# xuanjiangliu/robotic-discovery-platform

Hardware: AMD Instinct MI355X
Metric: U-Net train imgs/sec at 256×256 (1/2/4/8 GPU); e2e frames/sec + p50 latency (higher is better)
Workload: dtype bf16; 1 GPU; model=UNet(3,1) bilinear decoder, 17.26M params, global_batch=64, per_gpu_batch=64, image_size=256, parallelism=dp1, impl=native, optimizer=Adam(lr=1e-4), loss=bce, sync_bn=False, hipgraph=False

## Files before the change

### csrc/conv_wgrad.hip

```cpp
#include "common.h"
#include <algorithm>
#include <stdlib.h>
#include <string.h>

struct WgradArgs {
  const u16* x1;
  const u16* x2;
  uint32_t xbytes1, xbytes2;
  int C1, C2, pitch1, pitch2;
  const u16* dy;
  uint32_t dybytes;
  int dypitch;
  float* slab;
  int H, W, M, Cout, Cin;
  int taps, packed;
  int ncols, ncols_pad;
  int colTiles, coutTiles, splits;
  int pix_per_split;
  uint32_t fw_m, fw_s, fh_m, fh_s;
  int uH2 = 0, uW2 = 0, uoy = 0, uox = 0;
};

RDP_DEV int swz(int p) { return (((p >> 1) & 1) << 1) | (((p >> 3) & 1) << 2); }

// ... 582 lines not shown
  }
}


extern "C" int rdp_conv_wgrad(const void* x1, const void* x2, long xbytes1, long xbytes2, int C1, int C2, int pitch1,
                              int pitch2, const void* dy, long dybytes, int dypitch, float* slab, long slab_elems,
                              float* out, int accumulate, int N, int H, int W, int Cout, int taps, int packed,
                              int cin_real, int splits, int variant, hipStream_t s) {
  WgradArgs a;
  a.x1 = (const u16*)x1; a.x2 = (const u16*)x2;
  a.xbytes1 = (uint32_t)xbytes1; a.xbytes2 = (uint32_t)xbytes2;
  a.C1 = C1; a.C2 = C2; a.pitch1 = pitch1; a.pitch2 = pitch2;
  a.dy = (const u16*)dy; a.dybytes = (uint32_t)dybytes; a.dypitch = dypitch;
  a.slab = slab; a.H = H; a.W = W; a.M = N * H * W; a.Cout = Cout;
  a.taps = taps; a.packed = packed;
  if (packed) {
    if (C1 != 8 || C2 != 0 || taps != 9) return -1;
    a.Cin = 8; a.ncols = 72;
  } else {
    if (C1 % 64 || C2 % 64) return -1;
    a.Cin = C1 + C2; a.ncols = taps * a.Cin;
  }
  if (Cout % 64) return -1;
  if (xbytes1 >= (1l << 31) || xbytes2 >= (1l << 31) || dybytes >= (1l << 31)) return -1;
  const bool halo_ok = !packed && taps == 9 && (W % 64 == 0 || (W >= 32 && 64 % W == 0 && (H * W) % 64 == 0)) &&
                       variant != 4;
  if (variant == 5 && !(!packed && taps == 9 && (W % 64 == 0 || (W >= 8 && 64 % W == 0 && (H * W) % 64 == 0))))
    return -1;
  if (halo_ok || variant == 5) {
    WgradHaloArgs h;
    h.x1 = a.x1; h.x2 = a.x2; h.xbytes1 = a.xbytes1; h.xbytes2 = a.xbytes2;
    h.C1 = C1; h.C2 = C2; h.pitch1 = pitch1; h.pitch2 = pitch2;
    h.dy = a.dy; h.dybytes = a.dybytes; h.dypitch = dypitch;
    h.slab = slab; h.H = H; h.W = W; h.Cout = Cout; h.ncols = 9 * a.Cin;
    const int BN = Cout % 128 == 0 ? 128 : 64;
    h.cinTiles = a.Cin / 64; h.coutTiles = Cout / BN;
    const int tiles = h.cinTiles * h.coutTiles;
    h.nseg = a.M / 64;
    const int target = BN == 64 ? 512 : 256;
    int sp = std::max(1, (target + tiles - 1) / tiles);
    sp = std::min(sp, std::max(1, h.nseg));
    const long per_split = (long)Cout * h.ncols;
    sp = (int)std::min<long>(sp, slab_elems / per_split);
    if (sp < 1) return -2;
    h.segs_per_split = (h.nseg + sp - 1) / sp;
    h.splits = (h.nseg + h.segs_per_split - 1) / h.segs_per_split;
    if ((long)h.splits * per_split * 4l >= (1l << 31)) return -3;
    h.slab_bytes = (uint32_t)(h.splits * per_split * 4l);
    FastDiv fw = make_fastdiv(W), fh = make_fastdiv(H);
    h.fw_m = fw.m; h.fw_s = fw.s; h.fh_m = fh.m; h.fh_s = fh.s;
    const int nblk = tiles * h.splits;
    if (variant == 0 && W % 64 == 0 && BN == 64) {
      WgradRingArgs g;
      g.x1 = h.x1; g.x2 = h.x2; g.xbytes1 = h.xbytes1; g.xbytes2 = h.xbytes2;
      g.C1 = C1; g.C2 = C2; g.pitch1 = pitch1; g.pitch2 = pitch2;
      g.dy = h.dy; g.dybytes = h.dybytes; g.dypitch = dypitch;
      g.slab = slab; g.slab_bytes = h.slab_bytes; g.H = H; g.W = W; g.Cout = Cout; g.ncols = h.ncols;
      g.cinTiles = h.cinTiles; g.coutTiles = h.coutTiles; g.splits = h.splits;
      g.pos_per_split = h.segs_per_split; g.npos = h.nseg; g.WS = W / 64;
      FastDiv fs = make_fastdiv(W / 64);
      g.fh_m = fh.m; g.fh_s = fh.s; g.fs_m = fs.m; g.fs_s = fs.s;
      hipLaunchKernelGGL((conv_wgrad_ring_kernel<64>), dim3(nblk), dim3(256), 0, s, g);
    } else {
      const bool mr = W < 64;
      if (BN == 128 && mr) hipLaunchKernelGGL((conv_wgrad_halo_kernel<128, true>), dim3(nblk), dim3(512), 0, s, h);
      else if (BN == 128) hipLaunchKernelGGL((conv_wgrad_halo_kernel<128, false>), dim3(nblk), dim3(512), 0, s, h);
      else if (mr) hipLaunchKernelGGL((conv_wgrad_halo_kernel<64, true>), dim3(nblk), dim3(256), 0, s, h);
      else hipLaunchKernelGGL((conv_wgrad_halo_kernel<64, false>), dim3(nblk), dim3(256), 0, s, h);
    }
    rdp_wgrad_reduce(slab, out, h.splits, Cout, h.ncols, 9, a.Cin, a.Cin, accumulate, s);
    return h.splits;
  }
  a.colTiles = (a.ncols + 255) / 256;
  a.ncols_pad = a.colTiles * 256;
  a.coutTiles = Cout / 64;
  if (splits < 1) splits = 1;
  int pps = (a.M + splits - 1) / splits;
  pps = (pps + 63) / 64 * 64;
  a.pix_per_split = pps;
  a.splits = (a.M + pps - 1) / pps;
  if ((long)a.splits * Cout * a.ncols_pad > slab_elems) return -2;
  if ((long)a.splits * Cout * a.ncols_pad * 4l >= (1l << 31)) return -3;
  FastDiv fw = make_fastdiv(W), fh = make_fastdiv(H);
  a.fw_m = fw.m; a.fw_s = fw.s; a.fh_m = fh.m; a.fh_s = fh.s;
  const int nblk = a.colTiles * a.coutTiles * a.splits;
  if (packed) hipLaunchKernelGGL((conv_wgrad_kernel<true>), dim3(nblk), dim3(512), 0, s, a);
  else hipLaunchKernelGGL((conv_wgrad_kernel<false>), dim3(nblk), dim3(512), 0, s, a);
  rdp_wgrad_reduce(slab, out, a.splits, Cout, a.ncols_pad, taps, packed ? 8 : a.Cin, packed ? cin_real : a.Cin,
                   accumulate, s);
  return a.splits;
}

extern "C" int rdp_conv_wgrad_upT(const void* du, long dubytes, int C, int dupitch, int H2, int W2, int oy, int ox,
                                  const void* x, long xbytes, int Cin, int xpitch, int N, int h, int w, float* slab,
                                  long slab_elems, float* out, int accumulate, int splits, hipStream_t s) {
  if (C % 64 || Cin % 64 || oy < 0 || ox < 0 || 2 * h + oy > H2 || 2 * w + ox > W2) return -1;
  if (dubytes >= (1l << 31) || xbytes >= (1l << 31)) return -1;
  WgradArgs a;
  a.x1 = (const u16*)du; a.x2 = nullptr; a.xbytes1 = (uint32_t)dubytes; a.xbytes2 = 0;
  a.C1 = C; a.C2 = 0; a.pitch1 = dupitch; a.pitch2 = dupitch;
  a.dy = (const u16*)x; a.dybytes = (uint32_t)xbytes; a.dypitch = xpitch;
  a.slab = slab; a.H = h; a.W = w; a.M = N * h * w; a.Cout = Cin;
  a.taps = 4; a.packed = 0; a.Cin = C; a.ncols = 4 * C;
  a.uH2 = H2; a.uW2 = W2; a.uoy = oy; a.uox = ox;
  a.colTiles = (a.ncols + 255) / 256;
  a.ncols_pad = a.colTiles * 256;
  a.coutTiles = Cin / 64;
  if (splits < 1) splits = 1;
  int pps = (a.M + splits - 1) / splits;
  pps = (pps + 63) / 64 * 64;
  a.pix_per_split = pps;
  a.splits = (a.M + pps - 1) / pps;
  if ((long)a.splits * a.Cout * a.ncols_pad > slab_elems) return -2;
  if ((long)a.splits * a.Cout * a.ncols_pad * 4l >= (1l << 31)) return -3;
  FastDiv fw = make_fastdiv(w), fh = make_fastdiv(h);
  a.fw_m = fw.m; a.fw_s = fw.s; a.fh_m = fh.m; a.fh_s = fh.s;
  const int nblk = a.colTiles * a.coutTiles * a.splits;
  hipLaunchKernelGGL((conv_wgrad_kernel<false, true>), dim3(nblk), dim3(512), 0, s, a);
  rdp_wgrad_reduce(slab, out, a.splits, Cin, a.ncols_pad, 4, C, C, accumulate, s);
  return a.splits;
}

struct FirstWgradArgs {
  const u16* x;
  uint32_t xbytes;
  int xpitch;
  const u16* da;
  uint32_t dabytes;
  int dapitch;
  const u16* y;
  uint32_t ybytes;
  int ypitch;
  const float* coef;
  const float* coef2;
  float* slab;
  uint32_t slab_bytes;
  int H, W, M, pix_per_split;
  uint32_t fw_m, fw_s, fh_m, fh_s;
};
constexpr int FWG_NCOLS = 80;

RDP_DEV void fw_unpack8(const uint4& v, float* f) {
  const uint32_t w[4] = {v.x, v.y, v.z, v.w};
#pragma unroll
  for (int i = 0; i < 4; ++i) {
    f[2 * i] = __uint_as_float(w[i] << 16);
    f[2 * i + 1] = __uint_as_float(w[i] & 0xffff0000u);
  }
}

__global__ __launch_bounds__(256, 2) void wgrad_first_bn_kernel(const FirstWgradArgs a) {
  constexpr int SUB = 64 * 128;
  constexpr int BUF = 3 * SUB;
  __shared__ __attribute__((aligned(16))) char smem[2 * BUF];
  const int lane = threadIdx.x & 63;
  const int wave = __builtin_amdgcn_readfirstlane(threadIdx.x >> 6);
  const int split = (int)xcd_remap(blockIdx.x, gridDim.x);
  const int pbeg = split * a.pix_per_split;
  const int nks = max(0, min(a.M, pbeg + a.pix_per_split) - pbeg) / 64;
  const auto rx = make_rsrc(a.x, a.xbytes);
  const auto rda = make_rsrc(a.da, a.dabytes);
  const auto ry = make_rsrc(a.y, a.ybytes);

  const int tc = threadIdx.x & 7, tr0 = threadIdx.x >> 3;
  float ss[8], hh[8], cA[8], cB[8], cK[8];
#pragma unroll
  for (int k = 0; k < 8; ++k) {
    const int c = 8 * tc + k;
    ss[k] = a.coef[128 + c]; hh[k] = a.coef[192 + c];
    cA[k] = a.coef2[c]; cB[k] = a.coef2[64 + c]; cK[k] = a.coef2[128 + c];
  }
  uint4 vd[2], vy[2];
  auto load_dz = [&](int ks) {
#pragma unroll
    for (int u = 0; u < 2; ++u) {
      const int m = pbeg + ks * 64 + tr0 + 32 * u;
      vd[u] = bload16(rda, (uint32_t)(m * a.dapitch + 8 * tc) * 2u);
      vy[u] = bload16(ry, (uint32_t)(m * a.ypitch + 8 * tc) * 2u);
    }
  };
  auto store_dz = [&](char* buf) {
#pragma unroll
    for (int u = 0; u < 2; ++u) {
      const int p = tr0 + 32 * u;
      float fd[8], fy[8];
      fw_unpack8(vd[u], fd);
      fw_unpack8(vy[u], fy);
      uint32_t o[4];
#pragma unroll
      for (int k = 0; k < 8; k += 2) {
        const float g0 = fmaf(fy[k], ss[k], hh[k]) > 0.f ? fd[k] : 0.f;
        const float g1 = fmaf(fy[k + 1], ss[k + 1], hh[k + 1]) > 0.f ? fd[k + 1] : 0.f;
        o[k / 2] = pack2bf(fmaf(cA[k], g0, fmaf(cB[k], fy[k], cK[k])),
                           fmaf(cA[k + 1], g1, fmaf(cB[k + 1], fy[k + 1], cK[k + 1])));
      }
      *(uint4*)(buf + 2 * SUB + p * 128 + 16 * (tc ^ swz(p))) = make_uint4(o[0], o[1], o[2], o[3]);
    }
  };
  const int rowl = lane >> 3, cpos = lane & 7;
  auto issue_x = [&](int ks, char* buf) {
#pragma unroll
    for (int t = 0; t < 4; ++t) {
      const int s = wave * 4 + t, sub = s >> 3, pj = s & 7;
      const int p = pj * 8 + rowl;
      const int g = cpos ^ swz(p);
      const int m = pbeg + ks * 64 + p;
      const uint32_t q = fdiv2((uint32_t)m, a.fw_m, a.fw_s);
      const int w = m - (int)q * a.W;
      const int h = (int)q - (int)fdiv2(q, a.fh_m, a.fh_s) * a.H;
      const int tap = sub * 8 + g;
      const int dr = tap / 3 - 1, ds = tap % 3 - 1;
      const bool ok = (tap < 9) & inb(h + dr, a.H) & inb(w + ds, a.W);
      const uint32_t off = ok ? (uint32_t)((m + dr * a.W + ds) * a.xpitch) * 2u : RDP_OOB;
      dma16_async(rx, (lds_void*)(buf + sub * SUB + pj * 1024), off);
    }
  };

  f32x4 acc[5];
#pragma unroll
  for (int i = 0; i < 5; ++i) acc[i] = f32x4{0.f, 0.f, 0.f, 0.f};
  const int tg = lane >> 4, tq = (lane >> 2) & 3, tpp = lane & 3;
  typedef __attribute__((address_space(3))) bf16x4 lds_v4;

  if (nks > 0) {
    load_dz(0);
    issue_x(0, smem);
    store_dz(smem);
  }
  for (int ks = 0; ks < nks; ++ks) {
    asm volatile("s_waitcnt vmcnt(0) lgkmcnt(0)" ::: "memory");
    raw_barrier();
    const char* cur = smem + (ks & 1) * BUF;
    char* nxt = smem + ((ks + 1) & 1) * BUF;
    const bool more = ks + 1 < nks;
    if (more) {
      load_dz(ks + 1);
      issue_x(ks + 1, nxt);
    }
#pragma unroll
    for (int hf = 0; hf < 2; ++hf) {
      const int p0 = 32 * hf + 8 * tg + tq;
      const int sw0 = swz(p0), sw1 = swz(p0 + 4);
      const int ro0 = p0 * 128 + 8 * (tpp & 1), ro1 = ro0 + 4 * 128;
      auto frag = [&](const char* base, int i) {
        const int c = 2 * i + (tpp >> 1);
        const bf16x4 b0 = __builtin_amdgcn_ds_read_tr16_b64_v4i16((lds_v4*)(base + ro0 + 16 * (c ^ sw0)));
        const bf16x4 b1 = __builtin_amdgcn_ds_read_tr16_b64_v4i16((lds_v4*)(base + ro1 + 16 * (c ^ sw1)));
        return __builtin_shufflevector(b0, b1, 0, 1, 2, 3, 4, 5, 6, 7);
      };
      const bf16x8 fb = frag(cur + 2 * SUB, wave);
      bf16x8 fa[5];
#pragma unroll
      for (int i = 0; i < 4; ++i) fa[i] = frag(cur, i);
      fa[4] = frag(cur + SUB, 0);
#pragma unroll
      for (int i = 0; i < 5; ++i) acc[i] = __builtin_amdgcn_mfma_f32_16x16x32_bf16(fa[i], fb, acc[i], 0, 0, 0);
    }
    if (more) store_dz(nxt);
  }

  const auto rs = make_rsrc(a.slab, a.slab_bytes);
  const int co = 16 * wave + (lane & 15);
#pragma unroll
  for (int i = 0; i < 5; ++i) {
    const int col = 16 * i + 4 * (lane >> 4);
    const uint32_t off = (uint32_t)(((long)split * 64 + co) * FWG_NCOLS + col) * 4u;
    uint4 v;
    v.x = __float_as_uint(acc[i][0]); v.y = __float_as_uint(acc[i][1]);
    v.z = __float_as_uint(acc[i][2]); v.w = __float_as_uint(acc[i][3]);
    bstore16(rs, off, v);
  }
}

extern "C" int rdp_wgrad_first_bn(const void* x, long xbytes, int xpitch, const void* da, long dabytes, int dapitch,
                                  const void* y, long ybytes, int ypitch, const float* coef, const float* coef2,
                                  float* slab, long slab_elems, float* out, int accumulate, int N, int H, int W,
                                  int cin_real, int splits, hipStream_t s) {
  const long M = (long)N * H * W;
  if (M % 64 || cin_real > 8 || cin_real < 1) return -1;
  if (xbytes >= (1l << 31) || dabytes >= (1l << 31) || ybytes >= (1l << 31)) return -1;
  if (xpitch % 8 || dapitch % 8 || ypitch % 8) return -1;
  splits = (int)std::max(1L, std::min<long>(splits, M / 64));
  long pps = (M + splits - 1) / splits;
  pps = (pps + 63) / 64 * 64;
  splits = (int)((M + pps - 1) / pps);
  const long per_split = 64l * FWG_NCOLS;
  if ((long)splits * per_split > slab_elems) return -2;
  if ((long)splits * per_split * 4l >= (1l << 31)) return -3;
  FirstWgradArgs a;
  a.x = (const u16*)x; a.xbytes = (uint32_t)xbytes; a.xpitch = xpitch;
  a.da = (const u16*)da; a.dabytes = (uint32_t)dabytes; a.dapitch = dapitch;
  a.y = (const u16*)y; a.ybytes = (uint32_t)ybytes; a.ypitch = ypitch;
  a.coef = coef; a.coef2 = coef2;
  a.slab = slab; a.slab_bytes = (uint32_t)(splits * per_split * 4l);
  a.H = H; a.W = W; a.M = (int)M; a.pix_per_split = (int)pps;
  FastDiv fw = make_fastdiv(W), fh = make_fastdiv(H);
  a.fw_m = fw.m; a.fw_s = fw.s; a.fh_m = fh.m; a.fh_s = fh.s;
  hipLaunchKernelGGL(wgrad_first_bn_kernel, dim3(splits), dim3(256), 0, s, a);
  rdp_wgrad_reduce(slab, out, splits, 64, FWG_NCOLS, 9, 8, cin_real, accumulate, s);
  return splits;
}

extern "C" long rdp_conv_wgrad_slab_elems(int N, int H, int W, int Cin, int Cout, int taps, int packed, int splits) {
  const int ncols = packed ? 72 : taps * Cin;
  const int ncols_pad = (ncols + 255) / 256 * 256;
  const long M = (long)N * H * W;
  long pps = (M + splits - 1) / splits;
  pps = (pps + 63) / 64 * 64;
  const long sp = (M + pps - 1) / pps;
  return sp * Cout * ncols_pad;
}

extern "C" long rdp_conv_wgrad_halo_slab_elems(int N, int H, int W, int Cin, int Cout) {
  const long M = (long)N * H * W;
  const bool halo = Cin % 64 == 0 && Cout % 64 == 0 && (W % 64 == 0 || (W >= 32 && 64 % W == 0 && (H * W) % 64 == 0));
  if (!halo) return 0;
  const int BN = Cout % 128 == 0 ? 128 : 64;
  const long tiles = (long)(Cin / 64) * (Cout / BN);
  const long target = BN == 64 ? 512 : 256;
  long hsp = std::max<long>(1, (target + tiles - 1) / tiles);
  hsp = std::min<long>(hsp, std::max<long>(1, M / 64));
  return hsp * Cout * 9L * Cin;
}
```

### csrc/pool_up.hip

```cpp
#include "common.h"
#include <algorithm>

RDP_DEV void unpack8f(const uint4& v, float* f) {
  const uint32_t w[4] = {v.x, v.y, v.z, v.w};
#pragma unroll
  for (int k = 0; k < 4; ++k) {
    f[2 * k] = __uint_as_float(w[k] << 16);
    f[2 * k + 1] = __uint_as_float(w[k] & 0xffff0000u);
  }
}
RDP_DEV uint4 pack8f(const float* f) {
  uint4 v;
  v.x = pack2bf(f[0], f[1]);
  v.y = pack2bf(f[2], f[3]);
  v.z = pack2bf(f[4], f[5]);
  v.w = pack2bf(f[6], f[7]);
  return v;
}

__global__ void maxpool2_fwd_kernel(const u16* __restrict__ x, int xpitch, u16* __restrict__ out, int opitch, int N,
                                    int H, int W, int C) {
  const int Ho = H / 2, Wo = W / 2, CG = C >> 3;
  const long total = (long)N * Ho * Wo * CG;
  for (long it = blockIdx.x * (long)blockDim.x + threadIdx.x; it < total; it += (long)gridDim.x * blockDim.x) {
    const int g = it % CG;
    const long po = it / CG;
    const int wo = po % Wo;
    const long t = po / Wo;
    const int ho = t % Ho, n = t / Ho;
    const long p00 = ((long)n * H + 2 * ho) * W + 2 * wo;
    const int c = g * 8;
    float v[4][8];
    unpack8f(*(const uint4*)(x + p00 * xpitch + c), v[0]);
    unpack8f(*(const uint4*)(x + (p00 + 1) * xpitch + c), v[1]);
    unpack8f(*(const uint4*)(x + (p00 + W) * xpitch + c), v[2]);
    unpack8f(*(const uint4*)(x + (p00 + W + 1) * xpitch + c), v[3]);
    float o[8];
#pragma unroll
    for (int k = 0; k < 8; ++k) {
      float m = v[0][k];
#pragma unroll
      for (int q = 1; q < 4; ++q)
        if (v[q][k] > m || isnan(v[q][k])) m = v[q][k];
      o[k] = m;
    }
    *(uint4*)(out + po * opitch + c) = pack8f(o);
  }
}

__global__ void maxpool2_bwd_kernel(const u16* __restrict__ dp, int dppitch, const u16* __restrict__ x, int xpitch,
                                    const u16* __restrict__ dskip, int dspitch, u16* __restrict__ dx, int dxpitch,
                                    int N, int H, int W, int C) {
  const int Ho = H / 2, Wo = W / 2, CG = C >> 3;
  const int Hc = (H + 1) / 2, Wc = (W + 1) / 2;
  const long total = (long)N * Hc * Wc * CG;
  for (long it = blockIdx.x * (long)blockDim.x + threadIdx.x; it < total; it += (long)gridDim.x * blockDim.x) {
    const int g = it % CG;
    const long pw = it / CG;
    const int wc = pw % Wc;
    const long t = pw / Wc;
    const int hc = t % Hc, n = t / Hc;
    const int c = g * 8;
    const bool pooled = hc < Ho && wc < Wo;
    float v[4][8], d[8], o[4][8];
    int idx[8];
    if (pooled) {
      const long p00 = ((long)n * H + 2 * hc) * W + 2 * wc;
      unpack8f(*(const uint4*)(x + p00 * xpitch + c), v[0]);
      unpack8f(*(const uint4*)(x + (p00 + 1) * xpitch + c), v[1]);
      unpack8f(*(const uint4*)(x + (p00 + W) * xpitch + c), v[2]);
      unpack8f(*(const uint4*)(x + (p00 + W + 1) * xpitch + c), v[3]);
      const long po = ((long)n * Ho + hc) * Wo + wc;
      unpack8f(*(const uint4*)(dp + po * dppitch + c), d);
#pragma unroll
      for (int k = 0; k < 8; ++k) {
        float m = v[0][k];
        int id = 0;
#pragma unroll
        for (int q = 1; q < 4; ++q)
          if (v[q][k] > m || isnan(v[q][k])) { m = v[q][k]; id = q; }
        idx[k] = id;
      }
    }
#pragma unroll
    for (int q = 0; q < 4; ++q) {
      const int hh = 2 * hc + (q >> 1), ww = 2 * wc + (q & 1);
      if (hh >= H || ww >= W) continue;
      const long p = ((long)n * H + hh) * W + ww;
      float s[8];
      if (dskip) unpack8f(*(const uint4*)(dskip + p * dspitch + c), s);
      else {
#pragma unroll
        for (int k = 0; k < 8; ++k) s[k] = 0.f;
      }
#pragma unroll
      for (int k = 0; k < 8; ++k) o[q][k] = s[k] + ((pooled && idx[k] == q) ? d[k] : 0.f);
      *(uint4*)(dx + p * dxpitch + c) = pack8f(o[q]);
    }
  }
}

RDP_DEV void ld8f(const float* p, float* f) {
  const float4 a = *(const float4*)p, b = *(const float4*)(p + 4);
  f[0] = a.x; f[1] = a.y; f[2] = a.z; f[3] = a.w; f[4] = b.x; f[5] = b.y; f[6] = b.z; f[7] = b.w;
}

__global__ __launch_bounds__(256) void bn_relu_apply_pool_kernel(const u16* __restrict__ y, int ypitch,
                                                                 u16* __restrict__ a, int apitch,
                                                                 u16* __restrict__ pool, int ppitch,
                                                                 const float* __restrict__ coef, int N, int H, int W,
                                                                 int C) {
  const int CG = C >> 3, RPB = 256 / CG;
  const int g = threadIdx.x & (CG - 1), r = threadIdx.x / CG;
  const int c = g * 8;
  float ss[8], hh[8];
  ld8f(coef + 2 * C + c, ss);
  ld8f(coef + 3 * C + c, hh);
  const int Ho = H / 2, Wo = W / 2, Hc = (H + 1) / 2, Wc = (W + 1) / 2;
  const int nwin = N * Hc * Wc;
  for (int wi = blockIdx.x * RPB + r; wi < nwin; wi += gridDim.x * RPB) {
    const int wc = wi % Wc, t = wi / Wc;
    const int hc = t % Hc, n = t / Hc;
    uint4 v[4];
    bool ok[4];
    long px[4];
#pragma unroll
    for (int q = 0; q < 4; ++q) {
      const int h = 2 * hc + (q >> 1), w = 2 * wc + (q & 1);
      ok[q] = h < H && w < W;
      px[q] = ((long)n * H + h) * W + w;
      if (ok[q]) v[q] = *(const uint4*)(y + px[q] * ypitch + c);
    }
    float av[4][8];
#pragma unroll
    for (int q = 0; q < 4; ++q) {
      if (!ok[q]) continue;
      float f[8];
      unpack8f(v[q], f);
#pragma unroll
      for (int k = 0; k < 8; ++k) f[k] = fmaxf(fmaf(f[k], ss[k], hh[k]), 0.f);
      const uint4 o = pack8f(f);
      if (a) *(uint4*)(a + px[q] * apitch + c) = o;
      unpack8f(o, av[q]);
    }
    if (hc < Ho && wc < Wo) {
      float o[8];
#pragma unroll
      for (int k = 0; k < 8; ++k) {
        float m = av[0][k];
#pragma unroll
        for (int q = 1; q < 4; ++q)
          if (av[q][k] > m || isnan(av[q][k])) m = av[q][k];
        o[k] = m;
      }
      *(uint4*)(pool + (((long)n * Ho + hc) * Wo + wc) * ppitch + c) = pack8f(o);
    }
  }
}

__global__ __launch_bounds__(256) void maxpool2_bwd_bn_reduce_kernel(
    const u16* __restrict__ dp, int dppitch, const u16* __restrict__ dskip,
    int dspitch, u16* __restrict__ dx, int dxpitch, const u16* __restrict__ y, int ypitch,
    const float* __restrict__ coef, int N, int H, int W, int C, float* __restrict__ partial) {
  extern __shared__ __attribute__((aligned(16))) float sred[];
  const int CG = C >> 3, RPB = 256 / CG;
  const int g = threadIdx.x & (CG - 1), r = threadIdx.x / CG;
  const int c = g * 8;
  float mean[8], inv[8], ss[8], hh[8];
  ld8f(coef + c, mean);
  ld8f(coef + C + c, inv);
  ld8f(coef + 2 * C + c, ss);
  ld8f(coef + 3 * C + c, hh);
  float sg[8], sgx[8];
#pragma unroll
  for (int k = 0; k < 8; ++k) { sg[k] = 0.f; sgx[k] = 0.f; }
  const int Ho = H / 2, Wo = W / 2, Hc = (H + 1) / 2, Wc = (W + 1) / 2;
  const int nwin = N * Hc * Wc;
  for (int wi = blockIdx.x * RPB + r; wi < nwin; wi += gridDim.x * RPB) {
    const int wc = wi % Wc, t = wi / Wc;
    const int hc = t % Hc, n = t / Hc;
    const bool pooled = hc < Ho && wc < Wo;
    bool ok[4];
    long px[4];
    uint4 vs[4], vy[4], vd;
#pragma unroll
    for (int q = 0; q < 4; ++q) {
      const int h = 2 * hc + (q >> 1), w = 2 * wc + (q & 1);
      ok[q] = h < H && w < W;
      px[q] = ((long)n * H + h) * W + w;
      if (ok[q]) {
        vy[q] = *(const uint4*)(y + px[q] * ypitch + c);
        vs[q] = dskip ? *(const uint4*)(dskip + px[q] * dspitch + c) : make_uint4(0, 0, 0, 0);
      }
    }
    if (pooled) vd = *(const uint4*)(dp + (((long)n * Ho + hc) * Wo + wc) * dppitch + c);
    int idx[8];
    float d[8];
    if (pooled) {
      float v[4][8];
#pragma unroll
      for (int q = 0; q < 4; ++q) {
        float f[8];
        unpack8f(vy[q], f);
#pragma unroll
        for (int k = 0; k < 8; ++k) f[k] = fmaxf(fmaf(f[k], ss[k], hh[k]), 0.f);
        unpack8f(pack8f(f), v[q]);
      }
      unpack8f(vd, d);
#pragma unroll
      for (int k = 0; k < 8; ++k) {
        float m = v[0][k];
        int id = 0;
#pragma unroll
        for (int q = 1; q < 4; ++q)
          if (v[q][k] > m || isnan(v[q][k])) { m = v[q][k]; id = q; }
        idx[k] = id;
      }
    }
#pragma unroll
    for (int q = 0; q < 4; ++q) {
      if (!ok[q]) continue;
      float sk[8], o[8], fy[8];
      unpack8f(vs[q], sk);
#pragma unroll
      for (int k = 0; k < 8; ++k) o[k] = sk[k] + ((pooled && idx[k] == q) ? d[k] : 0.f);
      const uint4 ov = pack8f(o);
      *(uint4*)(dx + px[q] * dxpitch + c) = ov;
      unpack8f(ov, o);
      unpack8f(vy[q], fy);
#pragma unroll
      for (int k = 0; k < 8; ++k) {
        const float gg = fmaf(fy[k], ss[k], hh[k]) > 0.f ? o[k] : 0.f;
        sg[k] += gg;
        sgx[k] += gg * (fy[k] - mean[k]) * inv[k];
      }
    }
  }
#pragma unroll
  for (int k = 0; k < 8; ++k) {
    sred[(r * C + c + k) * 2] = sg[k];
    sred[(r * C + c + k) * 2 + 1] = sgx[k];
  }
  __syncthreads();
  for (int cc = threadIdx.x; cc < C; cc += 256) {
    float a0 = 0.f, a1 = 0.f;
    for (int q = 0; q < RPB; ++q) { a0 += sred[(q * C + cc) * 2]; a1 += sred[(q * C + cc) * 2 + 1]; }
    partial[(size_t)blockIdx.x * 2 * C + cc] = a0;
    partial[(size_t)blockIdx.x * 2 * C + C + cc] = a1;
  }
}

struct UpGeom {
  int N, hin, win, Hout, Wout, oy, ox, C;
  float rh, rw;
};

RDP_DEV void up_src(int u, int in, float r, int& i0, int& i1, float& l1) {
  const float s = r * (float)u;
  i0 = (int)s;
  i1 = i0 + (i0 < in - 1 ? 1 : 0);
  l1 = s - (float)i0;
}

RDP_DEV void bn_relu8(float* v, const float* sc, const float* sh) {
#pragma unroll
  for (int k = 0; k < 8; ++k) v[k] = bf2f(f2bf(fmaxf(fmaf(v[k], sc[k], sh[k]), 0.f)));
}

__global__ __launch_bounds__(256) void upsample2_fwd_taps_kernel(const u16* __restrict__ x, int xpitch,
                                                                 u16* __restrict__ out, int opitch, UpGeom g, int lcg,
                                                                 int nchunk, const float* __restrict__ coef) {
  const int CG = 1 << lcg;
  const int items = g.N * g.Hout * nchunk;
  for (int it = blockIdx.x; it < items; it += gridDim.x) {
    const int row = it / nchunk, q = it - row * nchunk;
    const int n = row / g.Hout, Y = row - n * g.Hout;
    const int t = q * 256 + threadIdx.x;
    const int X = t >> lcg, c = (t & (CG - 1)) * 8;
    if (X >= g.Wout) continue;
    const int uy = Y - g.oy, ux = X - g.ox;
    float o[8];
    if (uy < 0 || ux < 0 || uy >= 2 * g.hin || ux >= 2 * g.win) {
#pragma unroll
      for (int k = 0; k < 8; ++k) o[k] = 0.f;
    } else {
      int y0, y1, x0, x1;
      float ly, lx;
      up_src(uy, g.hin, g.rh, y0, y1, ly);
      up_src(ux, g.win, g.rw, x0, x1, lx);
      const long base = (long)n * g.hin;
      float a[8], b[8], cc[8], d[8];
      unpack8f(*(const uint4*)(x + ((base + y0) * g.win + x0) * xpitch + c), a);
      unpack8f(*(const uint4*)(x + ((base + y0) * g.win + x1) * xpitch + c), b);
      unpack8f(*(const uint4*)(x + ((base + y1) * g.win + x0) * xpitch + c), cc);
      unpack8f(*(const uint4*)(x + ((base + y1) * g.win + x1) * xpitch + c), d);
      if (coef) {
        float sc[8], sh[8];
#pragma unroll
        for (int k = 0; k < 8; ++k) { sc[k] = coef[2 * g.C + c + k]; sh[k] = coef[3 * g.C + c + k]; }
        bn_relu8(a, sc, sh); bn_relu8(b, sc, sh); bn_relu8(cc, sc, sh); bn_relu8(d, sc, sh);
      }
      const float hy = 1.f - ly, hx = 1.f - lx;
#pragma unroll
      for (int k = 0; k < 8; ++k) o[k] = hy * (hx * a[k] + lx * b[k]) + ly * (hx * cc[k] + lx * d[k]);
    }
    *(uint4*)(out + ((long)row * g.Wout + X) * opitch + c) = pack8f(o);
  }
}

RDP_DEV void up_hrow(const u16* __restrict__ x, long rowbase, int x0, int x1, int xpitch, int c, float hx,
                     float lx, const float* __restrict__ coef, int C, float* h) {
  float a[8], b[8];
  unpack8f(*(const uint4*)(x + (rowbase + x0) * xpitch + c), a);
  unpack8f(*(const uint4*)(x + (rowbase + x1) * xpitch + c), b);
  if (coef) {
    float sc[8], sh[8];
#pragma unroll
    for (int k = 0; k < 8; ++k) { sc[k] = coef[2 * C + c + k]; sh[k] = coef[3 * C + c + k]; }
    bn_relu8(a, sc, sh); bn_relu8(b, sc, sh);
  }
#pragma unroll
  for (int k = 0; k < 8; ++k) h[k] = hx * a[k] + lx * b[k];
}

__global__ __launch_bounds__(256) void upsample2_fwd_kernel(const u16* __restrict__ x, int xpitch,
                                                            u16* __restrict__ out, int opitch, UpGeom g, int lcg,
                                                            int nchunk, int R, const float* __restrict__ coef) {
  const int CG = 1 << lcg;
  const int nband = (g.Hout + R - 1) / R;
  const int items = g.N * nband * nchunk;
  for (int it = blockIdx.x; it < items; it += gridDim.x) {
    const int band = it / nchunk, q = it - band * nchunk;
    const int n = band / nband, Yb = (band - n * nband) * R;
    const int t = q * 256 + threadIdx.x;
    const int X = t >> lcg, c = (t & (CG - 1)) * 8;
    if (X >= g.Wout) continue;
    const int ux = X - g.ox;
    const bool xin = ux >= 0 && ux < 2 * g.win;
    int x0 = 0, x1 = 0;
    float lx = 0.f;
    if (xin) up_src(ux, g.win, g.rw, x0, x1, lx);
    const float hx = 1.f - lx;
    const long base = (long)n * g.hin;
    float h0[8], h1[8];
    int r0 = -1, r1 = -1;
    const int Ye = min(Yb + R, g.Hout);
    for (int Y = Yb; Y < Ye; ++Y) {
      const int uy = Y - g.oy;
      float o[8];
      if (!xin || uy < 0 || uy >= 2 * g.hin) {
#pragma unroll
        for (int k = 0; k < 8; ++k) o[k] = 0.f;
      } else {
        int y0, y1;
        float ly;
        up_src(uy, g.hin, g.rh, y0, y1, ly);
        if (y0 != r0) {
          if (y0 == r1) {
#pragma unroll
            for (int k = 0; k < 8; ++k) h0[k] = h1[k];
          } else {
            up_hrow(x, (base + y0) * g.win, x0, x1, xpitch, c, hx, lx, coef, g.C, h0);
          }
          r0 = y0;
        }
        if (y1 != r1) {
          if (y1 == r0) {
#pragma unroll
            for (int k = 0; k < 8; ++k) h1[k] = h0[k];
          } else {
            up_hrow(x, (base + y1) * g.win, x0, x1, xpitch, c, hx, lx, coef, g.C, h1);
          }
          r1 = y1;
        }
        const float hy = 1.f - ly;
#pragma unroll
        for (int k = 0; k < 8; ++k) o[k] = hy * h0[k] + ly * h1[k];
      }
      *(uint4*)(out + (((long)n * g.Hout + Y) * g.Wout + X) * opitch + c) = pack8f(o);
    }
  }
}

RDP_DEV float up_weight(int u, int in, float r, int i) {
  int i0, i1;
  float l1;
  up_src(u, in, r, i0, i1, l1);
  return (i0 == i ? 1.f - l1 : 0.f) + (i1 == i ? l1 : 0.f);
// ... 112 lines not shown
      partial[(size_t)blockIdx.x * 2 * g.C + cc] = a0;
      partial[(size_t)blockIdx.x * 2 * g.C + g.C + cc] = a1;
    }
  }
}

static int gridN(long items) {
  long g = (items + 255) / 256;
  return (int)std::max<long>(1, std::min<long>(g, 4096));
}
static float ac_scale(int in, int out) { return out > 1 ? (float)(in - 1) / (float)(out - 1) : 0.f; }

struct UpTGeom {
  int N, h, w, H2, W2, oy, ox, C;
};

__global__ void upT_shuffle_kernel(const u16* __restrict__ yT, int ypitch, const float* __restrict__ bias,
                                   u16* __restrict__ u, int upitch, UpTGeom g) {
  const int CG = g.C >> 3;
  const long total = (long)g.N * g.H2 * g.W2 * CG;
  for (long it = blockIdx.x * (long)blockDim.x + threadIdx.x; it < total; it += (long)gridDim.x * blockDim.x) {
    const int cg = (int)(it % CG);
    const long pix = it / CG;
    const int x = (int)(pix % g.W2);
    const long t = pix / g.W2;
    const int y = (int)(t % g.H2), n = (int)(t / g.H2);
    const int hy = y - g.oy, wx = x - g.ox;
    const int c = cg * 8;
    uint4 v = make_uint4(0u, 0u, 0u, 0u);
    if (hy >= 0 && hy < 2 * g.h && wx >= 0 && wx < 2 * g.w) {
      const long src = ((long)n * g.h + (hy >> 1)) * g.w + (wx >> 1);
      const int j = ((hy & 1) * 2 + (wx & 1)) * g.C + c;
      float f[8];
      unpack8f(*(const uint4*)(yT + src * ypitch + j), f);
#pragma unroll
      for (int k = 0; k < 8; ++k) f[k] += bias[c + k];
      v = pack8f(f);
    }
    *(uint4*)(u + pix * upitch + c) = v;
  }
}

__global__ void upT_unshuffle_kernel(const u16* __restrict__ du, int dpitch, u16* __restrict__ dyT, int ypitch,
                                     UpTGeom g) {
  const int CG4 = (4 * g.C) >> 3;
  const long total = (long)g.N * g.h * g.w * CG4;
  for (long it = blockIdx.x * (long)blockDim.x + threadIdx.x; it < total; it += (long)gridDim.x * blockDim.x) {
    const int jg = (int)(it % CG4);
    const long pix = it / CG4;
    const int ww = (int)(pix % g.w);
    const long t = pix / g.w;
    const int hh = (int)(t % g.h), n = (int)(t / g.h);
    const int j = jg * 8, sub = j / g.C, c = j - sub * g.C;
    const int y = 2 * hh + (sub >> 1) + g.oy, x = 2 * ww + (sub & 1) + g.ox;
    uint4 v = make_uint4(0u, 0u, 0u, 0u);
    if (y >= 0 && y < g.H2 && x >= 0 && x < g.W2) v = *(const uint4*)(du + (((long)n * g.H2 + y) * g.W2 + x) * dpitch + c);
    *(uint4*)(dyT + pix * ypitch + j) = v;
  }
}

__global__ __launch_bounds__(256) void colsum_bf16_kernel(const u16* __restrict__ x, int pitch, long M, int K,
                                                          float* __restrict__ partial) {
  extern __shared__ float sred2[];
  const int CG = K >> 3, RPB = 256 / CG;
  const int g = threadIdx.x % CG, r = threadIdx.x / CG;
  float acc[8];
#pragma unroll
  for (int k = 0; k < 8; ++k) acc[k] = 0.f;
  if (r < RPB)
    for (long p = blockIdx.x * (long)RPB + r; p < M; p += (long)gridDim.x * RPB) {
      float f[8];
      unpack8f(*(const uint4*)(x + p * pitch + g * 8), f);
#pragma unroll
      for (int k = 0; k < 8; ++k) acc[k] += f[k];
    }
  if (r < RPB)
#pragma unroll
    for (int k = 0; k < 8; ++k) sred2[r * K + g * 8 + k] = acc[k];
  __syncthreads();
  for (int cc = threadIdx.x; cc < K; cc += 256) {
    float s = 0.f;
    for (int q = 0; q < RPB; ++q) s += sred2[q * K + cc];
    partial[(long)blockIdx.x * K + cc] = s;
  }
}
constexpr int FOLD_RB = 32;
__global__ __launch_bounds__(256) void colsum_fold_kernel(const float* __restrict__ partial, int nblk, int K, int groups,
                                                          double* __restrict__ part2) {
  __shared__ double sfold[4][64];
  const int C = K / groups;
  const int tx = threadIdx.x & 63, ty = threadIdx.x >> 6;
  const int c = blockIdx.x * 64 + tx;
  const long rows = (long)nblk * groups;
  const long r0 = rows * blockIdx.y / FOLD_RB, r1 = rows * (blockIdx.y + 1) / FOLD_RB;
  double s0 = 0.0, s1 = 0.0, s2 = 0.0, s3 = 0.0;
  if (c < C) {
    long q = r0 + ty;
    for (; q + 12 < r1; q += 16) {
      const float v0 = partial[(q / groups) * K + (q % groups) * C + c];
      const float v1 = partial[((q + 4) / groups) * K + ((q + 4) % groups) * C + c];
      const float v2 = partial[((q + 8) / groups) * K + ((q + 8) % groups) * C + c];
      const float v3 = partial[((q + 12) / groups) * K + ((q + 12) % groups) * C + c];
      s0 += v0; s1 += v1; s2 += v2; s3 += v3;
    }
    for (; q < r1; q += 4) s0 += partial[(q / groups) * K + (q % groups) * C + c];
  }
  sfold[ty][tx] = (s0 + s1) + (s2 + s3);
  __syncthreads();
  if (ty == 0 && c < C) part2[(long)blockIdx.y * C + c] = ((sfold[0][tx] + sfold[1][tx]) + sfold[2][tx]) + sfold[3][tx];
}
__global__ __launch_bounds__(256) void colsum_fold2_kernel(const double* __restrict__ part2, int C, float* __restrict__ out,
                                                           int accumulate) {
  const int c = blockIdx.x * 256 + threadIdx.x;
  if (c >= C) return;
  double t = 0.0;
#pragma unroll
  for (int k = 0; k < FOLD_RB; ++k) t += part2[(long)k * C + c];
  out[c] = accumulate ? out[c] + (float)t : (float)t;
}


extern "C" {
int rdp_maxpool2_fwd(const void* x, int xpitch, void* out, int opitch, int N, int H, int W, int C, hipStream_t s) {
  if (C % 8 || xpitch % 8 || opitch % 8) return -1;
  hipLaunchKernelGGL(maxpool2_fwd_kernel, dim3(gridN((long)N * (H / 2) * (W / 2) * (C / 8))), dim3(256), 0, s,
                     (const u16*)x, xpitch, (u16*)out, opitch, N, H, W, C);
  return 0;
}
int rdp_maxpool2_bwd(const void* dp, int dppitch, const void* x, int xpitch, const void* dskip, int dspitch, void* dx,
                     int dxpitch, int N, int H, int W, int C, hipStream_t s) {
  if (C % 8) return -1;
  hipLaunchKernelGGL(maxpool2_bwd_kernel, dim3(gridN((long)N * ((H + 1) / 2) * ((W + 1) / 2) * (C / 8))), dim3(256),
                     0, s, (const u16*)dp, dppitch, (const u16*)x, xpitch, (const u16*)dskip, dspitch, (u16*)dx,
                     dxpitch, N, H, W, C);
  return 0;
}
static bool pow2c(int C) { return C >= 8 && C <= 2048 && (C & (C - 1)) == 0; }
int rdp_bn_relu_apply_pool(const void* y, int ypitch, void* a, int apitch, void* pool, int ppitch, const float* coef,
                           int N, int H, int W, int C, hipStream_t s) {
  if (!pow2c(C) || ypitch % 8 || apitch % 8 || ppitch % 8) return -1;
  const long rpb = 256 / (C / 8), nwin = (long)N * ((H + 1) / 2) * ((W + 1) / 2);
  const int grid = (int)std::max<long>(1, std::min<long>((nwin + rpb - 1) / rpb, 16384));
  hipLaunchKernelGGL(bn_relu_apply_pool_kernel, dim3(grid), dim3(256), 0, s, (const u16*)y, ypitch, (u16*)a, apitch,
                     (u16*)pool, ppitch, coef, N, H, W, C);
  return 0;
}
int rdp_maxpool2_bwd_bn_reduce(const void* dp, int dppitch, const void* x, int xpitch, const void* dskip, int dspitch,
                               void* dx, int dxpitch, const void* y, int ypitch, const float* coef, int N, int H, int W,
                               int C, float* partial, int max_blocks, hipStream_t s) {
  if (!pow2c(C) || dppitch % 8 || xpitch % 8 || dspitch % 8 || dxpitch % 8 || ypitch % 8) return -1;
  const long rpb = 256 / (C / 8), nwin = (long)N * ((H + 1) / 2) * ((W + 1) / 2);
  const int grid = (int)std::max<long>(1, std::min<long>((nwin + 4 * rpb - 1) / (4 * rpb), max_blocks));
  const size_t lds = (size_t)rpb * C * 2 * sizeof(float);
  hipLaunchKernelGGL(maxpool2_bwd_bn_reduce_kernel, dim3(grid), dim3(256), lds, s, (const u16*)dp, dppitch,
                     (const u16*)dskip, dspitch, (u16*)dx, dxpitch, (const u16*)y, ypitch, coef,
                     N, H, W, C, partial);
  return grid;
}
static int ilog2(int v) {
  int l = 0;
  while ((1 << l) < v) ++l;
  return l;
}
int rdp_upsample2_fwd(const void* x, int xpitch, void* out, int opitch, int N, int hin, int win, int Hout, int Wout,
                      int oy, int ox, int C, const float* coef, hipStream_t s) {
  if (!pow2c(C) || xpitch % 8 || opitch % 8) return -1;
  UpGeom g{N, hin, win, Hout, Wout, oy, ox, C, ac_scale(hin, 2 * hin), ac_scale(win, 2 * win)};
  const int lcg = ilog2(C / 8), nchunk = (int)(((long)Wout * (C / 8) + 255) / 256);
  int R = 8;
  while (R > 1 && (long)N * ((Hout + R - 1) / R) * nchunk < 4096) R >>= 1;
  const long items = (long)N * ((Hout + R - 1) / R) * nchunk;
  if (R == 1) {
    hipLaunchKernelGGL(upsample2_fwd_taps_kernel, dim3((int)std::min<long>(items, 8192)), dim3(256), 0, s,
                       (const u16*)x, xpitch, (u16*)out, opitch, g, lcg, nchunk, coef);
    return 0;
  }
  hipLaunchKernelGGL(upsample2_fwd_kernel, dim3((int)std::min<long>(items, 32768)), dim3(256), 0, s, (const u16*)x,
                     xpitch, (u16*)out, opitch, g, lcg, nchunk, R, coef);
  return 0;
}
int rdp_upsample2_bwd(const void* dout, int dpitch, void* dx, int xpitch, int N, int hin, int win, int Hout, int Wout,
                      int oy, int ox, int C, const void* y, int ypitch, const float* coef, float* partial,
                      int max_blocks, hipStream_t s) {
  if (!pow2c(C) || dpitch % 8 || xpitch % 8 || (y && ypitch % 8)) return -1;
  UpGeom g{N, hin, win, Hout, Wout, oy, ox, C, ac_scale(hin, 2 * hin), ac_scale(win, 2 * win)};
  const int lcg = ilog2(C / 8), nchunk = (int)(((long)win * (C / 8) + 255) / 256);
  int R = 4;
  while (R > 1 && (long)N * ((hin + R - 1) / R) * nchunk < 4096) R >>= 1;
  const long items = (long)N * ((hin + R - 1) / R) * nchunk;
  if (y) {
    const int grid = (int)std::max<long>(1, std::min<long>(items, max_blocks));
    const size_t lds = (size_t)(256 / (C / 8)) * C * 2 * sizeof(float);
    hipLaunchKernelGGL(upsample2_bwd_kernel<true>, dim3(grid), dim3(256), lds, s, (const u16*)dout, dpitch, (u16*)dx,
                       xpitch, g, lcg, nchunk, R, (const u16*)y, ypitch, coef, partial);
    return grid;
  }
  hipLaunchKernelGGL(upsample2_bwd_kernel<false>, dim3((int)std::min<long>(items, 8192)), dim3(256), 0, s,
                     (const u16*)dout, dpitch, (u16*)dx, xpitch, g, lcg, nchunk, R, (const u16*)nullptr, 0,
                     (const float*)nullptr, (float*)nullptr);
  return 0;
}
int rdp_upT_shuffle(const void* yT, int ypitch, const float* bias, void* u, int upitch, int N, int h, int w, int H2,
                    int W2, int oy, int ox, int C, hipStream_t s) {
  if (C % 8 || ypitch % 8 || upitch % 8) return -1;
  UpTGeom g{N, h, w, H2, W2, oy, ox, C};
  hipLaunchKernelGGL(upT_shuffle_kernel, dim3(gridN((long)N * H2 * W2 * (C / 8))), dim3(256), 0, s, (const u16*)yT,
                     ypitch, bias, (u16*)u, upitch, g);
  return 0;
}
int rdp_upT_unshuffle(const void* du, int dpitch, void* dyT, int ypitch, int N, int h, int w, int H2, int W2, int oy,
                      int ox, int C, hipStream_t s) {
  if (C % 8 || ypitch % 8 || dpitch % 8) return -1;
  UpTGeom g{N, h, w, H2, W2, oy, ox, C};
  hipLaunchKernelGGL(upT_unshuffle_kernel, dim3(gridN((long)N * h * w * (4 * C / 8))), dim3(256), 0, s,
                     (const u16*)du, dpitch, (u16*)dyT, ypitch, g);
  return 0;
}
int rdp_colsum_bf16(const void* x, int pitch, long M, int K, int groups, float* partial, float* out, int accumulate,
                    hipStream_t s) {
  if (K < 8 || K > 2048 || (K & (K - 1)) || K % groups || pitch % 8) return -1;
  const int rpb = 256 / (K / 8);
  const int nblk = (int)std::max<long>(1, std::min<long>(1024, (M + rpb * 16 - 1) / (rpb * 16)));
  hipLaunchKernelGGL(colsum_bf16_kernel, dim3(nblk), dim3(256), (size_t)rpb * K * sizeof(float), s, (const u16*)x,
                     pitch, M, K, partial);
  const int C = K / groups;
  double* part2 = (double*)(partial + 1024L * K);
  hipLaunchKernelGGL(colsum_fold_kernel, dim3((C + 63) / 64, FOLD_RB), dim3(256), 0, s, partial, nblk, K, groups, part2);
  hipLaunchKernelGGL(colsum_fold2_kernel, dim3((C + 255) / 256), dim3(256), 0, s, (const double*)part2, C, out, accumulate);
  return 0;
}
}
```

Before: 3414 images/s.

## Triple-buffer first-layer wgrad and software-pipeline maxpool backward window loads

The first-layer BN-fused weight-gradient kernel moves from two to three LDS buffers and prefetches two k-steps ahead, waiting with a partial vmcnt so the loads for the next step stay in flight across the barrier. The maxpool-backward BN-reduce kernel now loads the next window's data before reducing the current one. It also gets a template variant with the skip input compiled in or out, and out-of-bounds lanes use clamped or predicated loads. The aim is to hide global-memory latency behind compute, at the cost of more LDS per block (lower occupancy at launch bounds 2), more registers, and a hand-tuned wait count that must match the number of outstanding loads.

```diff
diff --git a/csrc/conv_wgrad.hip b/csrc/conv_wgrad.hip
--- a/csrc/conv_wgrad.hip
+++ b/csrc/conv_wgrad.hip
@@ -758,7 +758,7 @@
 __global__ __launch_bounds__(256, 2) void wgrad_first_bn_kernel(const FirstWgradArgs a) {
   constexpr int SUB = 64 * 128;
   constexpr int BUF = 3 * SUB;
-  __shared__ __attribute__((aligned(16))) char smem[2 * BUF];
+  __shared__ __attribute__((aligned(16))) char smem[3 * BUF];
   const int lane = threadIdx.x & 63;
   const int wave = __builtin_amdgcn_readfirstlane(threadIdx.x >> 6);
   const int split = (int)xcd_remap(blockIdx.x, gridDim.x);
@@ -776,22 +776,22 @@
     ss[k] = a.coef[128 + c]; hh[k] = a.coef[192 + c];
     cA[k] = a.coef2[c]; cB[k] = a.coef2[64 + c]; cK[k] = a.coef2[128 + c];
   }
-  uint4 vd[2], vy[2];
-  auto load_dz = [&](int ks) {
+  struct DzRegs { uint4 vd[2], vy[2]; };
+  auto load_dz = [&](int ks, DzRegs& z) {
 #pragma unroll
     for (int u = 0; u < 2; ++u) {
       const int m = pbeg + ks * 64 + tr0 + 32 * u;
-      vd[u] = bload16(rda, (uint32_t)(m * a.dapitch + 8 * tc) * 2u);
-      vy[u] = bload16(ry, (uint32_t)(m * a.ypitch + 8 * tc) * 2u);
+      z.vd[u] = bload16(rda, ks < nks ? (uint32_t)(m * a.dapitch + 8 * tc) * 2u : RDP_OOB);
+      z.vy[u] = bload16(ry, ks < nks ? (uint32_t)(m * a.ypitch + 8 * tc) * 2u : RDP_OOB);
     }
   };
-  auto store_dz = [&](char* buf) {
+  auto store_dz = [&](char* buf, const DzRegs& z) {
 #pragma unroll
     for (int u = 0; u < 2; ++u) {
       const int p = tr0 + 32 * u;
       float fd[8], fy[8];
-      fw_unpack8(vd[u], fd);
-      fw_unpack8(vy[u], fy);
+      fw_unpack8(z.vd[u], fd);
+      fw_unpack8(z.vy[u], fy);
       uint32_t o[4];
 #pragma unroll
       for (int k = 0; k < 8; k += 2) {
@@ -816,7 +816,7 @@
       const int h = (int)q - (int)fdiv2(q, a.fh_m, a.fh_s) * a.H;
       const int tap = sub * 8 + g;
       const int dr = tap / 3 - 1, ds = tap % 3 - 1;
-      const bool ok = (tap < 9) & inb(h + dr, a.H) & inb(w + ds, a.W);
+      const bool ok = (ks < nks) & (tap < 9) & inb(h + dr, a.H) & inb(w + ds, a.W);
       const uint32_t off = ok ? (uint32_t)((m + dr * a.W + ds) * a.xpitch) * 2u : RDP_OOB;
       dma16_async(rx, (lds_void*)(buf + sub * SUB + pj * 1024), off);
     }
@@ -828,21 +828,20 @@
   const int tg = lane >> 4, tq = (lane >> 2) & 3, tpp = lane & 3;
   typedef __attribute__((address_space(3))) bf16x4 lds_v4;
 
+  DzRegs z0, z1;
   if (nks > 0) {
-    load_dz(0);
     issue_x(0, smem);
-    store_dz(smem);
-  }
-  for (int ks = 0; ks < nks; ++ks) {
-    asm volatile("s_waitcnt vmcnt(0) lgkmcnt(0)" ::: "memory");
+    load_dz(0, z0);
+    issue_x(1, smem + BUF);
+    load_dz(1, z1);
+    store_dz(smem, z0);
+  }
+  auto kstep = [&](int ks, const char* cur, char* nxt, char* far, DzRegs& zs, const DzRegs& zn) {
+    asm volatile("s_waitcnt vmcnt(12) lgkmcnt(0)" ::: "memory");
     raw_barrier();
-    const char* cur = smem + (ks & 1) * BUF;
-    char* nxt = smem + ((ks + 1) & 1) * BUF;
     const bool more = ks + 1 < nks;
-    if (more) {
-      load_dz(ks + 1);
-      issue_x(ks + 1, nxt);
-    }
+    issue_x(ks + 2, far);
+    load_dz(ks + 2, zs);
 #pragma unroll
     for (int hf = 0; hf < 2; ++hf) {
       const int p0 = 32 * hf + 8 * tg + tq;
@@ -862,7 +861,20 @@
 #pragma unroll
       for (int i = 0; i < 5; ++i) acc[i] = __builtin_amdgcn_mfma_f32_16x16x32_bf16(fa[i], fb, acc[i], 0, 0, 0);
     }
-    if (more) store_dz(nxt);
+    if (more) store_dz(nxt, zn);
+  };
+  char* b0 = smem;
+  char* b1 = smem + BUF;
+  char* b2 = smem + 2 * BUF;
+  for (int ks = 0; ks < nks;) {
+    kstep(ks, b0, b1, b2, z0, z1);
+    if (++ks >= nks) break;
+    kstep(ks, b1, b2, b0, z1, z0);
+    ++ks;
+    char* t = b0;
+    b0 = b2;
+    b2 = b1;
+    b1 = t;
   }
 
   const auto rs = make_rsrc(a.slab, a.slab_bytes);
diff --git a/csrc/pool_up.hip b/csrc/pool_up.hip
--- a/csrc/pool_up.hip
+++ b/csrc/pool_up.hip
@@ -158,6 +158,7 @@
   }
 }
 
+template <bool SKIP>
 __global__ __launch_bounds__(256) void maxpool2_bwd_bn_reduce_kernel(
     const u16* __restrict__ dp, int dppitch, const u16* __restrict__ dskip,
     int dspitch, u16* __restrict__ dx, int dxpitch, const u16* __restrict__ y, int ypitch,
@@ -176,24 +177,30 @@
   for (int k = 0; k < 8; ++k) { sg[k] = 0.f; sgx[k] = 0.f; }
   const int Ho = H / 2, Wo = W / 2, Hc = (H + 1) / 2, Wc = (W + 1) / 2;
   const int nwin = N * Hc * Wc;
-  for (int wi = blockIdx.x * RPB + r; wi < nwin; wi += gridDim.x * RPB) {
+  struct Win {
+    uint4 vs[4], vy[4], vd;
+    long px0;
+    bool okh, okw;
+  };
+  const bool anyp = Ho > 0 && Wo > 0;
+  const u16* dpb = anyp ? dp : y;
+  auto load_win = [&](int wi, Win& w) {
     const int wc = wi % Wc, t = wi / Wc;
     const int hc = t % Hc, n = t / Hc;
-    const bool pooled = hc < Ho && wc < Wo;
-    bool ok[4];
-    long px[4];
-    uint4 vs[4], vy[4], vd;
+    w.okh = hc < Ho;
+    w.okw = wc < Wo;
+    w.px0 = ((long)n * H + 2 * hc) * W + 2 * wc;
 #pragma unroll
     for (int q = 0; q < 4; ++q) {
-      const int h = 2 * hc + (q >> 1), w = 2 * wc + (q & 1);
-      ok[q] = h < H && w < W;
-      px[q] = ((long)n * H + h) * W + w;
-      if (ok[q]) {
-        vy[q] = *(const uint4*)(y + px[q] * ypitch + c);
-        vs[q] = dskip ? *(const uint4*)(dskip + px[q] * dspitch + c) : make_uint4(0, 0, 0, 0);
-      }
-    }
-    if (pooled) vd = *(const uint4*)(dp + (((long)n * Ho + hc) * Wo + wc) * dppitch + c);
+      const long px = w.px0 + (w.okh ? (q >> 1) * W : 0) + (w.okw ? (q & 1) : 0);
+      w.vy[q] = *(const uint4*)(y + px * ypitch + c);
+      w.vs[q] = SKIP ? *(const uint4*)(dskip + px * dspitch + c) : make_uint4(0, 0, 0, 0);
+    }
+    const long pc = anyp ? (((long)n * Ho + min(hc, Ho - 1)) * Wo + min(wc, Wo - 1)) * dppitch + c : 0;
+    w.vd = *(const uint4*)(dpb + pc);
+  };
+  auto reduce_win = [&](const Win& w) {
+    const bool pooled = w.okh && w.okw;
     int idx[8];
     float d[8];
     if (pooled) {
@@ -201,12 +208,12 @@
 #pragma unroll
       for (int q = 0; q < 4; ++q) {
         float f[8];
-        unpack8f(vy[q], f);
+        unpack8f(w.vy[q], f);
 #pragma unroll
         for (int k = 0; k < 8; ++k) f[k] = fmaxf(fmaf(f[k], ss[k], hh[k]), 0.f);
         unpack8f(pack8f(f), v[q]);
       }
-      unpack8f(vd, d);
+      unpack8f(w.vd, d);
 #pragma unroll
       for (int k = 0; k < 8; ++k) {
         float m = v[0][k];
@@ -219,21 +226,38 @@
     }
 #pragma unroll
     for (int q = 0; q < 4; ++q) {
-      if (!ok[q]) continue;
+      if (!(((q >> 1) == 0 || w.okh) && ((q & 1) == 0 || w.okw))) continue;
+      const long px = w.px0 + (q >> 1) * W + (q & 1);
       float sk[8], o[8], fy[8];
-      unpack8f(vs[q], sk);
+      unpack8f(w.vs[q], sk);
 #pragma unroll
       for (int k = 0; k < 8; ++k) o[k] = sk[k] + ((pooled && idx[k] == q) ? d[k] : 0.f);
       const uint4 ov = pack8f(o);
-      *(uint4*)(dx + px[q] * dxpitch + c) = ov;
+      *(uint4*)(dx + px * dxpitch + c) = ov;
       unpack8f(ov, o);
-      unpack8f(vy[q], fy);
+      unpack8f(w.vy[q], fy);
 #pragma unroll
       for (int k = 0; k < 8; ++k) {
         const float gg = fmaf(fy[k], ss[k], hh[k]) > 0.f ? o[k] : 0.f;
         sg[k] += gg;
-        sgx[k] += gg * (fy[k] - mean[k]) * inv[k];
-      }
+        sgx[k] = fmaf(gg * (fy[k] - mean[k]), inv[k], sgx[k]);
+      }
+    }
+  };
+  const int step = gridDim.x * RPB;
+  int wi = blockIdx.x * RPB + r;
+  if (wi < nwin) {
+    Win w0, w1;
+    load_win(wi, w0);
+    for (;;) {
+      wi += step;
+      if (wi >= nwin) { reduce_win(w0); break; }
+      load_win(wi, w1);
+      reduce_win(w0);
+      wi += step;
+      if (wi >= nwin) { reduce_win(w1); break; }
+      load_win(wi, w0);
+      reduce_win(w1);
     }
   }
 #pragma unroll
@@ -652,7 +676,8 @@
   const long rpb = 256 / (C / 8), nwin = (long)N * ((H + 1) / 2) * ((W + 1) / 2);
   const int grid = (int)std::max<long>(1, std::min<long>((nwin + 4 * rpb - 1) / (4 * rpb), max_blocks));
   const size_t lds = (size_t)rpb * C * 2 * sizeof(float);
-  hipLaunchKernelGGL(maxpool2_bwd_bn_reduce_kernel, dim3(grid), dim3(256), lds, s, (const u16*)dp, dppitch,
+  auto kern = dskip ? maxpool2_bwd_bn_reduce_kernel<true> : maxpool2_bwd_bn_reduce_kernel<false>;
+  hipLaunchKernelGGL(kern, dim3(grid), dim3(256), lds, s, (const u16*)dp, dppitch,
                      (const u16*)dskip, dspitch, (u16*)dx, dxpitch, (const u16*)y, ypitch, coef,
                      N, H, W, C, partial);
   return grid;
```

Measured after the change: 3406 images/s. About the same (-0.2%).
